# jabberjabberjabber/video-3d-pipeline

Hardware: AMD Instinct MI355X
Metric: 1080p_sbs_to_4k_depth_frames_per_s (higher is better)
Workload: dtype int16 (SGM) + f64 (guided filter sums; f32 depth in/out)

## Files before the change

video-3d-pipeline_amd/csrc/v3d_guided.hip:

```cpp
#include "v3d_common.h"
#include <type_traits>

__device__ __forceinline__ double gf_rcp(double x)
{
    double r = __builtin_amdgcn_rcp(x);
    r = fma(r, fma(-x, r, 1.0), r);
    r = fma(r, fma(-x, r, 1.0), r);
    return r;
}

template <typename TD> __device__ __forceinline__ float gf_ld(const TD* p, size_t i);
template <> __device__ __forceinline__ float gf_ld<float>(const float* p, size_t i) { return p[i]; }
template <> __device__ __forceinline__ float gf_ld<int16_t>(const int16_t* p, size_t i) { const int d = p[i]; return d > 0 ? (float)d * 0.0625f : 0.f; }

#define GF_TX 64
#define GF_RUN 8
#define GF_RMAX 16

template <typename TD>
__device__ __forceinline__ double gf_bilinear(const TD* __restrict__ src, int Ws, int Hs, double sx, double sy, int x, int y)
{
    const double fx = (x + 0.5) * sx - 0.5, fy = (y + 0.5) * sy - 0.5;
    const double x0f = floor(fx), y0f = floor(fy);
    const double wx = fx - x0f, wy = fy - y0f;
// ... 99 lines not shown
            }
            if (j + 1 < GF_RUNY) {
                const int kn = j + 2 * r + 1;
#pragma unroll
                for (int q = 0; q < NS; q++) s[q] += h[q * hplane + kn * hp] - h[q * hplane + j * hp];
            }
        }
    }
}

#ifndef GF_CH
#define GF_CH 3
#endif
typedef double v3d_f64x2 __attribute__((ext_vector_type(2)));
typedef float v3d_f32x2 __attribute__((ext_vector_type(2)));

template <int SWEEP, int RR, typename TD>
__global__ __launch_bounds__(256) void k_gfm(const TD* __restrict__ depth_lo, int Wlo, int Hlo,
                                             const uint8_t* __restrict__ guide, int W, int H, double eps, int band_h,
                                             double* __restrict__ A, double* __restrict__ B, float* __restrict__ out,
                                             size_t depth_stride, size_t guide_stride)
{
    static_assert(RR % 2 == 0, "pairs must not straddle the strip's halo boundary");
    constexpr int R = 2 * RR + 1, NOUT = 256 - 2 * RR;
    __shared__ __attribute__((aligned(16))) double sVd[2][2][2][256];
    __shared__ __attribute__((aligned(16))) int2 sVi[2][2][256];
    {
        const size_t f = blockIdx.z, n4 = (size_t)W * H;
        depth_lo += f * depth_stride; guide += f * guide_stride; A += f * 2 * n4; B += f * 2 * n4; out += f * n4;
    }
// ... 154 lines not shown
                                v3d_f32x2 vq = { qa, qb };
                                __builtin_nontemporal_store(vq, reinterpret_cast<v3d_f32x2*>(out + o));
                            } else {
                                out[o] = qa;
                                if (px1) out[o + 1] = qb;
                            }
                        }
                    }
                    buf ^= 1;
                }
            }
        }
    }
}

__device__ __forceinline__ double gf_partner(double v)
{
    const int lo = __builtin_amdgcn_update_dpp(0, __double2loint(v), V3D_DPP_QUAD(1, 0, 3, 2), 0xF, 0xF, true);
    const int hi = __builtin_amdgcn_update_dpp(0, __double2hiint(v), V3D_DPP_QUAD(1, 0, 3, 2), 0xF, 0xF, true);
    return __hiloint2double(hi, lo);
}
__device__ __forceinline__ int gf_partner(int v) { return __builtin_amdgcn_update_dpp(0, v, V3D_DPP_QUAD(1, 0, 3, 2), 0xF, 0xF, true); }

template <int RR, int COLS, typename TD, bool I1>
__global__ __launch_bounds__(2 * COLS, 4) void k_gff(const TD* __restrict__ depth_lo, int Wlo, int Hlo,
                                                const uint8_t* __restrict__ guide, int W, int H, double eps, int band_h,
                                                float* __restrict__ out, size_t depth_stride, size_t guide_stride)
{
    static_assert(RR % 2 == 0, "pairs must not straddle the strip's halo boundaries");
    static_assert(!I1 || std::is_same<TD, int16_t>::value, "the integer stage 1 takes the int16 disparity");
    constexpr int R = 2 * RR + 1, NOUT = COLS - 4 * RR, HP = COLS / 2;
    static_assert(COLS == 256 || COLS == 512, "strip width");
    constexpr int S1D = 2 * 2 * 2 * COLS * 8, S1I = 2 * 2 * COLS * 8;
    __shared__ __attribute__((aligned(16))) unsigned char sS1[I1 ? 2 * 2 * COLS * 16 : S1D + S1I];
    double (*sV1)[2][2][COLS] = reinterpret_cast<double (*)[2][2][COLS]>(sS1);
    int2 (*sVi)[2][COLS] = reinterpret_cast<int2 (*)[2][COLS]>(sS1 + (I1 ? 0 : S1D));
    int4 (*sVq)[2][COLS] = reinterpret_cast<int4 (*)[2][COLS]>(sS1);
    (void)sV1; (void)sVi; (void)sVq;
    __shared__ __attribute__((aligned(16))) double sAB[2][2][2][COLS];
    __shared__ __attribute__((aligned(16))) double sV2[2][2][2][COLS];
    __shared__ __attribute__((aligned(16))) double sP2[2][2][2][COLS / 2];
    __shared__ __attribute__((aligned(16))) int4 sPq[I1 ? 2 : 1][2][I1 ? COLS / 2 : 1];
    (void)sPq;
    {
        const size_t f = blockIdx.z, n4 = (size_t)W * H;
        depth_lo += f * depth_stride; guide += f * guide_stride; out += f * n4;
    }
    const int role = __builtin_amdgcn_readfirstlane((int)(threadIdx.x / COLS));
    const int t = threadIdx.x % COLS;
    const int gx0 = blockIdx.x * NOUT - 2 * RR;
    const int gx = gx0 + t;
    const int ya = blockIdx.y * band_h, yb = min(ya + band_h, H);
    const int nrows = (yb - ya) + 4 * RR;
    const int NS = (nrows + 1) >> 1;
    const int NP = NS + 3;
    const int hq = t % HP, hgx = gx0 + 2 * hq;

    for (int i = threadIdx.x; i < 2 * 2 * 2 * COLS; i += 2 * COLS) (&sAB[0][0][0][0])[i] = 0.0;
    __syncthreads();

    if (role == 0) {
      if constexpr (I1) {
        const bool col_ok = gx >= 0 && gx < W;
        const bool pair_in = 2 * hq >= RR && 2 * hq < COLS - RR;
        const bool px0 = pair_in && hgx >= 0 && hgx < W, px1 = pair_in && hgx + 1 >= 0 && hgx + 1 < W;
        const int kx = gx >> 1;
        const int bxa = min(max((gx & 1) ? kx : kx - 1, 0), Wlo - 1), bxb = min(max((gx & 1) ? kx + 1 : kx, 0), Wlo - 1);
        const int wxa = (gx & 1) ? 3 : 1, wxb = 4 - wxa;
        uint32_t ring[R];
        int vg = 0, vgg = 0, vP = 0, vgP = 0;
#pragma unroll
        for (int j = 0; j < R; j++) ring[j] = 0u;
        struct RowIn { int g, a0, a1, b0, b1; bool in; };
        const int gxc = min(max(gx, 0), W - 1);
        auto fetch_row = [&](int tt) -> RowIn {
            RowIn q;
            const int e = ya - 2 * RR + tt;
            q.in = col_ok && e >= 0 && e < H && tt < nrows;
            const int ec = min(max(e, 0), H - 1), ky = ec >> 1;
            q.g = guide[(size_t)ec * W + gxc];
            const TD* ra = depth_lo + (size_t)min(max((ec & 1) ? ky : ky - 1, 0), Hlo - 1) * Wlo;
            const TD* rb = depth_lo + (size_t)min(max((ec & 1) ? ky + 1 : ky, 0), Hlo - 1) * Wlo;
            q.a0 = max((int)ra[bxa], 0); q.a1 = max((int)ra[bxb], 0); q.b0 = max((int)rb[bxa], 0); q.b1 = max((int)rb[bxb], 0);
            return q;
        };
        RowIn nx[2] = { fetch_row(0), fetch_row(1) };
        for (int p0 = 0; p0 < NP; p0 += R) {
#pragma unroll
            for (int sp = 0; sp < R; sp++) {
                const int p = p0 + sp;
                if (p < NP) {
                    int tl = t;
                    asm volatile("" : "+v"(tl));
                    const int hrow = tl / HP, hq = tl % HP, hgx = gx0 + 2 * hq;
                    const int j = p - 1;
                    if (j >= RR && j < NS && pair_in) {
                        const int hb = j & 1;
                        const int y = ya - 3 * RR + 2 * j + hrow;
                        double ab[2][2] = { { 0.0, 0.0 }, { 0.0, 0.0 } };
                        if (y >= 0 && y < H && px0) {
                            const int4* gp = &sPq[hb][hrow][hq - RR / 2];
                            const int4 f = sVq[hb][hrow][2 * hq - RR], l = sVq[hb][hrow][2 * hq + RR + 1];
                            int4 c = make_int4(0, 0, 0, 0);
#pragma unroll
                            for (int ch = 0; ch <= RR; ch += 3) {
                                int4 u[3];
#pragma unroll
                                for (int i = 0; i < 3; i++) if (ch + i <= RR) u[i] = gp[ch + i];
#pragma unroll
                                for (int i = 0; i < 3; i++) if (ch + i <= RR) { c.x += u[i].x; c.y += u[i].y; c.z += u[i].z; c.w += u[i].w; }
                                asm volatile("" : "+v"(c.x), "+v"(c.y), "+v"(c.z), "+v"(c.w) :: "memory");
                            }
                            const int cy = min(y + RR, H - 1) - max(y - RR, 0) + 1;
                            const int cx0 = min(hgx + RR, W - 1) - max(hgx - RR, 0) + 1, cx1 = min(hgx + 1 + RR, W - 1) - max(hgx + 1 - RR, 0) + 1;
                            const double inva = gf_rcp((double)(cx0 * cy)), invb = cx1 == cx0 ? inva : gf_rcp((double)(cx1 * cy));
#pragma unroll
                            for (int n = 0; n < 2; n++) {
                                const int4 e = n ? f : l;
                                const double inv = n ? invb : inva;
                                const double s0 = (double)(c.z - e.z) * (1.0 / 256.0), s1 = (double)(c.w - e.w) * (1.0 / 256.0);
                                const double mI = (double)(c.x - e.x) * (inv * (1.0 / 255.0)), mp = s0 * inv;
                                const double mII = (double)(c.y - e.y) * (inv * (1.0 / 65025.0)), mIp = s1 * (inv * (1.0 / 255.0));
                                const double var = fma(-mI, mI, mII), cov = fma(-mI, mp, mIp);
                                const double a = cov * gf_rcp(var + eps);
                                ab[n][0] = a; ab[n][1] = fma(-a, mI, mp);
                            }
                            if (!px1) { ab[1][0] = 0.0; ab[1][1] = 0.0; }
                        }
                        const v3d_f64x2 va2 = { ab[0][0], ab[1][0] }, vb2 = { ab[0][1], ab[1][1] };
                        *reinterpret_cast<v3d_f64x2*>(&sAB[hb][hrow][0][2 * hq]) = va2;
                        *reinterpret_cast<v3d_f64x2*>(&sAB[hb][hrow][1][2 * hq]) = vb2;
                    }
                    if (p < NS) {
                        const int tA = 2 * p;
                        const RowIn cur[2] = { nx[0], nx[1] };
                        nx[0] = fetch_row(tA + 2); nx[1] = fetch_row(tA + 3);
                        const bool emit = p >= RR;
#pragma unroll
                        for (int rr = 0; rr < 2; rr++) {
                            const int slot = (2 * sp + rr) % R;
                            int gn = 0, Pn = 0;
                            if (cur[rr].in) {
                                gn = cur[rr].g;
                                const int e = ya - 2 * RR + tA + rr;
                                const int wya = (e & 1) ? 3 : 1;
                                Pn = wya * (wxa * cur[rr].a0 + wxb * cur[rr].a1) + (4 - wya) * (wxa * cur[rr].b0 + wxb * cur[rr].b1);
                            }
                            const int go = (int)(ring[slot] & 0xFFu), Po = (int)(ring[slot] >> 8);
                            ring[slot] = ((uint32_t)Pn << 8) | (uint32_t)gn;
                            vg += gn - go; vgg += gn * gn - go * go;
                            vP += Pn - Po; vgP += gn * Pn - go * Po;
                            if (emit) {
                                sVq[p & 1][rr][t] = make_int4(vg, vgg, vP, vgP);
                                const int4 ps = make_int4(vg + gf_partner(vg), vgg + gf_partner(vgg), vP + gf_partner(vP), vgP + gf_partner(vgP));
                                if (!(t & 1)) sPq[p & 1][rr][t >> 1] = ps;
                            }
                        }
                    }
                    __syncthreads();
                }
            }
        }
      } else {
        const bool col_ok = gx >= 0 && gx < W;
        const double sx = (double)Wlo / (double)W, sy = (double)Hlo / (double)H;
        const bool pair_in = 2 * hq >= RR && 2 * hq < COLS - RR;
        const bool px0 = pair_in && hgx >= 0 && hgx < W, px1 = pair_in && hgx + 1 >= 0 && hgx + 1 < W;
        int bxa, bxb; double bwx;
        {
            const double fx = (gx + 0.5) * sx - 0.5, x0f = floor(fx);
            bwx = fx - x0f;
            bxa = min(max((int)x0f, 0), Wlo - 1); bxb = min(max((int)x0f + 1, 0), Wlo - 1);
        }
        double r1[R], v0 = 0.0, v1 = 0.0;
        uint32_t rgw[(R + 3) / 4];
        int vg = 0, vgg = 0;
#pragma unroll
        for (int j = 0; j < R; j++) r1[j] = 0.0;
#pragma unroll
        for (int j = 0; j < (R + 3) / 4; j++) rgw[j] = 0u;
        struct RowIn { int g; float a0, a1, b0, b1; bool in; };
        const int gxc = min(max(gx, 0), W - 1);
        auto fetch_row = [&](int tt) -> RowIn {
            RowIn q;
            const int e = ya - 2 * RR + tt;
            q.in = col_ok && e >= 0 && e < H && tt < nrows;
            const size_t o = (size_t)min(max(e, 0), H - 1) * W + gxc;
            q.g = guide[o];
            const double fy = (e + 0.5) * sy - 0.5, y0f = floor(fy);
            const TD* ra = depth_lo + (size_t)min(max((int)y0f, 0), Hlo - 1) * Wlo;
            const TD* rb = depth_lo + (size_t)min(max((int)y0f + 1, 0), Hlo - 1) * Wlo;
            q.a0 = gf_ld(ra, bxa); q.a1 = gf_ld(ra, bxb); q.b0 = gf_ld(rb, bxa); q.b1 = gf_ld(rb, bxb);
            return q;
        };
        RowIn nx[2] = { fetch_row(0), fetch_row(1) };
        for (int p0 = 0; p0 < NP; p0 += R) {
#pragma unroll
            for (int sp = 0; sp < R; sp++) {
                const int p = p0 + sp;
                if (p < NP) {
                    int tl = t;
                    asm volatile("" : "+v"(tl));
                    const int hrow = tl / HP, hq = tl % HP, hgx = gx0 + 2 * hq;
                    const int j = p - 1;
                    if (j >= RR && j < NS && pair_in) {
                        const int hb = j & 1;
                        const int y = ya - 3 * RR + 2 * j + hrow;
                        double ab[2][2] = { { 0.0, 0.0 }, { 0.0, 0.0 } };
                        if (y >= 0 && y < H && px0) {
                            double fq[2], lq[2], cq[2];
#pragma unroll
                            for (int q = 0; q < 2; q++) {
                                const v3d_f64x2* d = reinterpret_cast<const v3d_f64x2*>(&sV1[hb][hrow][q][0]) + (hq - RR / 2);
                                double f = 0.0, l = 0.0, c = 0.0;
#pragma unroll
                                for (int ch = 0; ch <= RR; ch += GF_CH) {
                                    v3d_f64x2 w[GF_CH];
#pragma unroll
                                    for (int i = 0; i < GF_CH; i++) if (ch + i <= RR) w[i] = d[ch + i];
#pragma unroll
                                    for (int i = 0; i < GF_CH; i++) if (ch + i <= RR) {
                                        if (ch + i == 0) { f = w[i].x; c = w[i].y; }
                                        else if (ch + i == RR) { c += w[i].x; l = w[i].y; }
                                        else { c += w[i].x; c += w[i].y; }
                                    }
                                    asm volatile("" : "+v"(c) :: "memory");
                                }
                                fq[q] = f; lq[q] = l; cq[q] = c;
                            }
                            int g0 = 0, gg0 = 0, gl = 0, ggl = 0, cg = 0, cgg = 0;
                            {
                                const int4* gi = reinterpret_cast<const int4*>(&sVi[hb][hrow][0]) + (hq - RR / 2);
#pragma unroll
                                for (int ch = 0; ch <= RR; ch += 3) {
                                    int4 u[3];
#pragma unroll
                                    for (int i = 0; i < 3; i++) if (ch + i <= RR) u[i] = gi[ch + i];
#pragma unroll
                                    for (int i = 0; i < 3; i++) if (ch + i <= RR) {
                                        if (ch + i == 0) { g0 = u[i].x; gg0 = u[i].y; cg = u[i].z; cgg = u[i].w; }
                                        else if (ch + i == RR) { cg += u[i].x; cgg += u[i].y; gl = u[i].z; ggl = u[i].w; }
                                        else { cg += u[i].x + u[i].z; cgg += u[i].y + u[i].w; }
                                    }
                                    asm volatile("" : "+v"(cg), "+v"(cgg) :: "memory");
                                }
                            }
                            const double s0a = cq[0] + fq[0], s0b = cq[0] + lq[0], s1a = cq[1] + fq[1], s1b = cq[1] + lq[1];
                            const int cy = min(y + RR, H - 1) - max(y - RR, 0) + 1;
                            const int cx0 = min(hgx + RR, W - 1) - max(hgx - RR, 0) + 1, cx1 = min(hgx + 1 + RR, W - 1) - max(hgx + 1 - RR, 0) + 1;
                            const double inva = gf_rcp((double)(cx0 * cy)), invb = cx1 == cx0 ? inva : gf_rcp((double)(cx1 * cy));
                            const int sga = cg + g0, sgb = cg + gl, sgga = cgg + gg0, sggb = cgg + ggl;
#pragma unroll
                            for (int n = 0; n < 2; n++) {
                                const double inv = n ? invb : inva;
                                const double mI = (double)(n ? sgb : sga) * (inv * (1.0 / 255.0)), mp = (n ? s0b : s0a) * inv;
                                const double mII = (double)(n ? sggb : sgga) * (inv * (1.0 / 65025.0)), mIp = (n ? s1b : s1a) * (inv * (1.0 / 255.0));
                                const double var = fma(-mI, mI, mII), cov = fma(-mI, mp, mIp);
                                const double a = cov * gf_rcp(var + eps);
                                ab[n][0] = a; ab[n][1] = fma(-a, mI, mp);
                            }
                            if (!px1) { ab[1][0] = 0.0; ab[1][1] = 0.0; }
                        }
                        const v3d_f64x2 va2 = { ab[0][0], ab[1][0] }, vb2 = { ab[0][1], ab[1][1] };
                        *reinterpret_cast<v3d_f64x2*>(&sAB[hb][hrow][0][2 * hq]) = va2;
                        *reinterpret_cast<v3d_f64x2*>(&sAB[hb][hrow][1][2 * hq]) = vb2;
                    }
                    if (p < NS) {
                        const int tA = 2 * p;
                        const RowIn cur[2] = { nx[0], nx[1] };
                        nx[0] = fetch_row(tA + 2); nx[1] = fetch_row(tA + 3);
                        const bool emit = p >= RR;
#pragma unroll
                        for (int rr = 0; rr < 2; rr++) {
                            const int slot = (2 * sp + rr) % R;
                            int gn = 0; double pn = 0.0;
                            if (cur[rr].in) {
                                gn = cur[rr].g;
                                const int e = ya - 2 * RR + tA + rr;
                                const double fy = (e + 0.5) * sy - 0.5, wy = fy - floor(fy);
                                const double a0 = (double)cur[rr].a0, b0 = (double)cur[rr].b0;
                                const double top = fma(bwx, (double)cur[rr].a1 - a0, a0);
                                const double bot = fma(bwx, (double)cur[rr].b1 - b0, b0);
                                pn = fma(wy, bot - top, top);
                            }
                            const int go = (int)((rgw[slot >> 2] >> (8 * (slot & 3))) & 0xFFu); const double po = r1[slot];
                            rgw[slot >> 2] = (rgw[slot >> 2] & ~(0xFFu << (8 * (slot & 3)))) | ((uint32_t)gn << (8 * (slot & 3)));
                            r1[slot] = pn;
                            vg += gn - go; vgg += gn * gn - go * go;
                            v0 += pn - po; v1 = fma((double)gn, pn, fma(-(double)go, po, v1));
                            if (emit) {
                                sV1[p & 1][rr][0][t] = v0; sV1[p & 1][rr][1][t] = v1;
                                sVi[p & 1][rr][t] = make_int2(vg, vgg);
                            }
                        }
                    }
                    __syncthreads();
                }
            }
        }
      }
    } else {
        const bool pair_out = 2 * hq >= 2 * RR && 2 * hq < COLS - 2 * RR;
        const bool px0 = pair_out && hgx < W, px1 = pair_out && hgx + 1 < W;
        const bool vec_ok = px1 && (W & 1) == 0;
        double r0[R], r1[R], va = 0.0, vb = 0.0;
#pragma unroll
        for (int j = 0; j < R; j++) { r0[j] = 0.0; r1[j] = 0.0; }
        for (int p0 = 0; p0 < NP; p0 += R) {
#pragma unroll
            for (int sp = 0; sp < R; sp++) {
                const int p = p0 + sp;
                if (p < NP) {
                    int tl = t;
                    asm volatile("" : "+v"(tl));
                    const int hrow = tl / HP, hq = tl % HP, hgx = gx0 + 2 * hq;
                    {
                        const int j = p - 3;
                        const int y = ya - 4 * RR + 2 * j + hrow;
                        if (j >= 2 * RR && j < NS && px0 && y < yb) {
                            const int hb = j & 1;
                            double wa[2], wb[2];
#pragma unroll
                            for (int q = 0; q < 2; q++) {
                                const double* d = &sP2[hb][hrow][q][hq - RR / 2];
                                const double f = sV2[hb][hrow][q][2 * hq - RR], l = sV2[hb][hrow][q][2 * hq + RR + 1];
                                double c = 0.0;
#pragma unroll
                                for (int ch = 0; ch <= RR; ch += 3) {
                                    double w[3];
#pragma unroll
                                    for (int i = 0; i < 3; i++) if (ch + i <= RR) w[i] = d[ch + i];
#pragma unroll
                                    for (int i = 0; i < 3; i++) if (ch + i <= RR) c += w[i];
                                    asm volatile("" : "+v"(c) :: "memory");
                                }
                                wa[q] = c - l; wb[q] = c - f;
                                asm volatile("" : "+v"(wa[q]), "+v"(wb[q]) :: "memory");
                            }
                            const double s0a = wa[0], s0b = wb[0], s1a = wa[1], s1b = wb[1];
                            const int cy = min(y + RR, H - 1) - max(y - RR, 0) + 1;
                            const int cx0 = min(hgx + RR, W - 1) - max(hgx - RR, 0) + 1, cx1 = min(hgx + 1 + RR, W - 1) - max(hgx + 1 - RR, 0) + 1;
                            const double inva = gf_rcp((double)(cx0 * cy)), invb = cx1 == cx0 ? inva : gf_rcp((double)(cx1 * cy));
                            const size_t o = (size_t)y * W + hgx;
                            const double Ia = (double)guide[o] * (1.0 / 255.0);
                            const double Ib = px1 ? (double)guide[o + 1] * (1.0 / 255.0) : 0.0;
                            const float qa = (float)((s0a * inva) * Ia + (s1a * inva)), qb = (float)((s0b * invb) * Ib + (s1b * invb));
                            if (vec_ok) {
                                v3d_f32x2 vq = { qa, qb };
                                __builtin_nontemporal_store(vq, reinterpret_cast<v3d_f32x2*>(out + o));
                            } else {
                                out[o] = qa;
                                if (px1) out[o + 1] = qb;
                            }
                        }
                    }
                    {
                        const int j = p - 2;
                        if (j >= RR && j < NS) {
                            const bool emit = j >= 2 * RR;
#pragma unroll
                            for (int rr = 0; rr < 2; rr++) {
                                const int slot = (2 * sp + rr) % R;
                                const double n0 = sAB[j & 1][rr][0][tl], n1 = sAB[j & 1][rr][1][tl];
                                const double o0 = r0[slot], o1 = r1[slot];
                                r0[slot] = n0; r1[slot] = n1;
                                va += n0 - o0; vb += n1 - o1;
                                if (emit) {
                                    sV2[j & 1][rr][0][tl] = va; sV2[j & 1][rr][1][tl] = vb;
                                    const double pa = va + gf_partner(va), pb = vb + gf_partner(vb);
                                    if (!(tl & 1)) { sP2[j & 1][rr][0][tl >> 1] = pa; sP2[j & 1][rr][1][tl >> 1] = pb; }
                                }
                            }
                        }
                    }
                    __syncthreads();
                }
            }
        }
    }
}

template <int RR, typename TD>
static void launch_gff(const TD* depth_lo, int Wlo, int Hlo, const uint8_t* guide, int W, int H, double eps,
                       float* out, int n, size_t depth_stride, size_t guide_stride, hipStream_t st)
{
    const int cols = g_v3d_opt.gf_cols == 512 ? 512 : 256;
    int band = g_v3d_opt.gf_band;
    if (band <= 0) {
        int dev = 0, ncu = 256;
        (void)hipGetDevice(&dev);
        (void)hipDeviceGetAttribute(&ncu, hipDeviceAttributeMultiprocessorCount, dev);
        const long slots = (long)ncu * (cols == 512 ? 1 : 2), strips = v3d_cdiv(W, cols - 4 * RR);
        long best = -1;
        for (int nb = 1; nb <= 64 && nb <= H; nb++) {
            const int b = (v3d_cdiv(H, nb) + 1) & ~1;
            const long wgs = strips * v3d_cdiv(H, b) * n, rounds = (wgs + slots - 1) / slots, cost = rounds * (b + 4 * RR);
            if (best < 0 || cost < best) { best = cost; band = b; }
        }
    }
    if (g_v3d_opt.gf_cols == 512) {
        const dim3 grid(v3d_cdiv(W, 512 - 4 * RR), v3d_cdiv(H, band), n);
        hipLaunchKernelGGL((k_gff<RR, 512, TD, false>), grid, dim3(1024), 0, st, depth_lo, Wlo, Hlo, guide, W, H, eps, band, out, depth_stride, guide_stride);
        return;
    }
    const dim3 grid(v3d_cdiv(W, 256 - 4 * RR), v3d_cdiv(H, band), n);
    if constexpr (std::is_same<TD, int16_t>::value) {
        if (g_v3d_opt.gf_int1 && W == 2 * Wlo && H == 2 * Hlo) {
            hipLaunchKernelGGL((k_gff<RR, 256, TD, true>), grid, dim3(512), 0, st, depth_lo, Wlo, Hlo, guide, W, H, eps, band, out, depth_stride, guide_stride);
            return;
        }
    }
    hipLaunchKernelGGL((k_gff<RR, 256, TD, false>), grid, dim3(512), 0, st, depth_lo, Wlo, Hlo, guide, W, H, eps, band, out, depth_stride, guide_stride);
}

template <int RR, typename TD>
static void launch_gfm(const TD* depth_lo, int Wlo, int Hlo, const uint8_t* guide, int W, int H, double eps,
                       double* A, double* B, float* out, int n, size_t depth_stride, size_t guide_stride, hipStream_t st)
{
    const int band1 = g_v3d_opt.gf_band1, band2 = g_v3d_opt.gf_band2;
    const dim3 grid1(v3d_cdiv(W, 256 - 2 * RR), v3d_cdiv(H, band1), n), grid2(v3d_cdiv(W, 256 - 2 * RR), v3d_cdiv(H, band2), n);
    hipLaunchKernelGGL((k_gfm<1, RR, TD>), grid1, dim3(256), 0, st, depth_lo, Wlo, Hlo, guide, W, H, eps, band1, A, B, out, depth_stride, guide_stride);
    hipLaunchKernelGGL((k_gfm<2, RR, TD>), grid2, dim3(256), 0, st, depth_lo, Wlo, Hlo, guide, W, H, eps, band2, A, B, out, depth_stride, guide_stride);
// ... 79 lines not shown
```

Measured before the change: 2485.

## Process four rows and four-pixel runs per step in fused guided filter

Restructures the fused guided-filter kernel so each step handles four rows and each thread computes a run of four horizontal box sums, using swizzled LDS layouts to avoid bank conflicts. The paired DPP partner-sum scheme and the separate sV2/sP2 buffers are replaced by a triple-buffered sAB array reused in place. The aim is fewer barriers per row and fewer LDS reads per output. It costs more registers and LDS, lowers the occupancy hint for the f64 route, and limits 512-column strips to the integer path.

```diff
diff --git a/video-3d-pipeline_amd/csrc/v3d_guided.hip b/video-3d-pipeline_amd/csrc/v3d_guided.hip
--- a/video-3d-pipeline_amd/csrc/v3d_guided.hip
+++ b/video-3d-pipeline_amd/csrc/v3d_guided.hip
@@ -137,6 +137,7 @@
 #endif
 typedef double v3d_f64x2 __attribute__((ext_vector_type(2)));
 typedef float v3d_f32x2 __attribute__((ext_vector_type(2)));
+typedef float v3d_f32x4 __attribute__((ext_vector_type(4)));
 
 template <int SWEEP, int RR, typename TD>
 __global__ __launch_bounds__(256) void k_gfm(const TD* __restrict__ depth_lo, int Wlo, int Hlo,
@@ -321,34 +322,128 @@
     }
 }
 
-__device__ __forceinline__ double gf_partner(double v)
-{
-    const int lo = __builtin_amdgcn_update_dpp(0, __double2loint(v), V3D_DPP_QUAD(1, 0, 3, 2), 0xF, 0xF, true);
-    const int hi = __builtin_amdgcn_update_dpp(0, __double2hiint(v), V3D_DPP_QUAD(1, 0, 3, 2), 0xF, 0xF, true);
-    return __hiloint2double(hi, lo);
-}
-__device__ __forceinline__ int gf_partner(int v) { return __builtin_amdgcn_update_dpp(0, v, V3D_DPP_QUAD(1, 0, 3, 2), 0xF, 0xF, true); }
+__device__ __forceinline__ int gf_swz2(int m) { return m ^ ((m >> 3) & 1) ^ ((m >> 4) & 1); }
+__device__ __forceinline__ int gf_swz4(int m) { return m ^ ((m >> 4) & 3); }
+__device__ __forceinline__ int gf_c8(int c) { return 2 * gf_swz2(c >> 1) + (c & 1); }
+
+template <int RR>
+__device__ __forceinline__ void gf_run4(const double* row, int c0, double s[4])
+{
+    const v3d_f64x2* d = reinterpret_cast<const v3d_f64x2*>(row);
+    const int m0 = (c0 - RR) >> 1;
+    double c = 0.0, l0 = 0.0, l1 = 0.0, l2 = 0.0, r1 = 0.0, r2 = 0.0, r3 = 0.0;
+#pragma unroll
+    for (int k0 = 0; k0 < RR + 2; k0 += GF_CH) {
+        v3d_f64x2 w[GF_CH];
+#pragma unroll
+        for (int i = 0; i < GF_CH; i++) if (k0 + i < RR + 2) w[i] = d[gf_swz2(m0 + k0 + i)];
+#pragma unroll
+        for (int i = 0; i < GF_CH; i++) {
+            const int k = k0 + i;
+            if (k == 0) { l0 = w[i].x; l1 = w[i].y; c = w[i].x; c += w[i].y; }
+            else if (k == 1) { l2 = w[i].x; c += w[i].x; c += w[i].y; }
+            else if (k < RR) { c += w[i].x; c += w[i].y; }
+            else if (k == RR) { c += w[i].x; r1 = w[i].y; }
+            else if (k == RR + 1) { r2 = w[i].x; r3 = w[i].y; }
+        }
+        asm volatile("" : "+v"(c) :: "memory");
+    }
+    s[0] = c; s[1] = (s[0] + r1) - l0; s[2] = (s[1] + r2) - l1; s[3] = (s[2] + r3) - l2;
+}
+
+template <int RR>
+__device__ __forceinline__ void gf_run4(const int2* row, int c0, int2 s[4])
+{
+    const int4* d = reinterpret_cast<const int4*>(row);
+    const int m0 = (c0 - RR) >> 1;
+    int2 c = make_int2(0, 0), l0 = c, l1 = c, l2 = c, r1 = c, r2 = c, r3 = c;
+#pragma unroll
+    for (int k0 = 0; k0 < RR + 2; k0 += 3) {
+        int4 w[3];
+#pragma unroll
+        for (int i = 0; i < 3; i++) if (k0 + i < RR + 2) w[i] = d[gf_swz2(m0 + k0 + i)];
+#pragma unroll
+        for (int i = 0; i < 3; i++) {
+            const int k = k0 + i;
+            const int2 a = make_int2(w[i].x, w[i].y), b = make_int2(w[i].z, w[i].w);
+            if (k == 0) { l0 = a; l1 = b; c = make_int2(a.x + b.x, a.y + b.y); }
+            else if (k == 1) { l2 = a; c.x += a.x + b.x; c.y += a.y + b.y; }
+            else if (k < RR) { c.x += a.x + b.x; c.y += a.y + b.y; }
+            else if (k == RR) { c.x += a.x; c.y += a.y; r1 = b; }
+            else if (k == RR + 1) { r2 = a; r3 = b; }
+        }
+        asm volatile("" : "+v"(c.x), "+v"(c.y) :: "memory");
+    }
+    s[0] = c;
+    s[1] = make_int2(s[0].x + r1.x - l0.x, s[0].y + r1.y - l0.y);
+    s[2] = make_int2(s[1].x + r2.x - l1.x, s[1].y + r2.y - l1.y);
+    s[3] = make_int2(s[2].x + r3.x - l2.x, s[2].y + r3.y - l2.y);
+}
+
+template <int RR>
+__device__ __forceinline__ void gf_run4(const int4* row, int c0, int4 s[4])
+{
+    int4 c = make_int4(0, 0, 0, 0), l0 = c, l1 = c, l2 = c, r1 = c, r2 = c, r3 = c;
+#pragma unroll
+    for (int k0 = 0; k0 < 2 * RR + 4; k0 += 3) {
+        int4 u[3];
+#pragma unroll
+        for (int i = 0; i < 3; i++) if (k0 + i < 2 * RR + 4) u[i] = row[gf_swz4(c0 - RR + k0 + i)];
+#pragma unroll
+        for (int i = 0; i < 3; i++) {
+            const int k = k0 + i;
+            if (k < 2 * RR + 1) { c.x += u[i].x; c.y += u[i].y; c.z += u[i].z; c.w += u[i].w; }
+            if (k == 0) l0 = u[i];
+            else if (k == 1) l1 = u[i];
+            else if (k == 2) l2 = u[i];
+            else if (k == 2 * RR + 1) r1 = u[i];
+            else if (k == 2 * RR + 2) r2 = u[i];
+            else if (k == 2 * RR + 3) r3 = u[i];
+        }
+        asm volatile("" : "+v"(c.x), "+v"(c.y), "+v"(c.z), "+v"(c.w) :: "memory");
+    }
+    s[0] = c;
+    s[1] = make_int4(s[0].x + r1.x - l0.x, s[0].y + r1.y - l0.y, s[0].z + r1.z - l0.z, s[0].w + r1.w - l0.w);
+    s[2] = make_int4(s[1].x + r2.x - l1.x, s[1].y + r2.y - l1.y, s[1].z + r2.z - l1.z, s[1].w + r2.w - l1.w);
+    s[3] = make_int4(s[2].x + r3.x - l2.x, s[2].y + r3.y - l2.y, s[2].z + r3.z - l2.z, s[2].w + r3.w - l2.w);
+}
+
+template <int RR>
+__device__ __forceinline__ void gf_solve4(const int sg[4], const int sgg[4], const double sp[4], const double sgp[4], int hgx, int y,
+                                          int W, int H, double eps, double a[4], double b[4])
+{
+    const int cy = min(y + RR, H - 1) - max(y - RR, 0) + 1;
+    int cx[4];
+#pragma unroll
+    for (int n = 0; n < 4; n++) cx[n] = min(hgx + n + RR, W - 1) - max(hgx + n - RR, 0) + 1;
+    const double inv0 = gf_rcp((double)(cx[0] * cy));
+#pragma unroll
+    for (int n = 0; n < 4; n++) {
+        const double inv = (n == 0 || cx[n] == cx[0]) ? inv0 : gf_rcp((double)(cx[n] * cy));
+        const double mI = (double)sg[n] * (inv * (1.0 / 255.0)), mp = sp[n] * inv;
+        const double mII = (double)sgg[n] * (inv * (1.0 / 65025.0)), mIp = sgp[n] * (inv * (1.0 / 255.0));
+        const double var = fma(-mI, mI, mII), cov = fma(-mI, mp, mIp);
+        const double aa = cov * gf_rcp(var + eps);
+        a[n] = aa; b[n] = fma(-aa, mI, mp);
+    }
+}
 
 template <int RR, int COLS, typename TD, bool I1>
-__global__ __launch_bounds__(2 * COLS, 4) void k_gff(const TD* __restrict__ depth_lo, int Wlo, int Hlo,
+__global__ __launch_bounds__(2 * COLS, I1 ? 4 : 2) void k_gff(const TD* __restrict__ depth_lo, int Wlo, int Hlo,
                                                 const uint8_t* __restrict__ guide, int W, int H, double eps, int band_h,
                                                 float* __restrict__ out, size_t depth_stride, size_t guide_stride)
 {
-    static_assert(RR % 2 == 0, "pairs must not straddle the strip's halo boundaries");
+    static_assert(RR % 4 == 0, "runs of four must not straddle the strip's halo boundaries");
     static_assert(!I1 || std::is_same<TD, int16_t>::value, "the integer stage 1 takes the int16 disparity");
-    constexpr int R = 2 * RR + 1, NOUT = COLS - 4 * RR, HP = COLS / 2;
-    static_assert(COLS == 256 || COLS == 512, "strip width");
-    constexpr int S1D = 2 * 2 * 2 * COLS * 8, S1I = 2 * 2 * COLS * 8;
-    __shared__ __attribute__((aligned(16))) unsigned char sS1[I1 ? 2 * 2 * COLS * 16 : S1D + S1I];
-    double (*sV1)[2][2][COLS] = reinterpret_cast<double (*)[2][2][COLS]>(sS1);
-    int2 (*sVi)[2][COLS] = reinterpret_cast<int2 (*)[2][COLS]>(sS1 + (I1 ? 0 : S1D));
-    int4 (*sVq)[2][COLS] = reinterpret_cast<int4 (*)[2][COLS]>(sS1);
+    static_assert(COLS == 256 || (COLS == 512 && I1), "strip width (512 columns: I1 only, the f64 route's rows exceed the LDS)");
+    constexpr int R = 2 * RR + 1, NOUT = COLS - 4 * RR, HR = COLS / 4;
+    constexpr int S1D = 2 * 4 * 2 * COLS * 8, S1 = I1 ? 2 * 4 * COLS * 16 : S1D + 2 * 4 * COLS * 8;
+    __shared__ __attribute__((aligned(16))) unsigned char sS1[S1];
+    double (*sV1)[4][2][COLS] = reinterpret_cast<double (*)[4][2][COLS]>(sS1);
+    int2 (*sVi)[4][COLS] = reinterpret_cast<int2 (*)[4][COLS]>(sS1 + (I1 ? 0 : S1D));
+    int4 (*sVq)[4][COLS] = reinterpret_cast<int4 (*)[4][COLS]>(sS1);
     (void)sV1; (void)sVi; (void)sVq;
-    __shared__ __attribute__((aligned(16))) double sAB[2][2][2][COLS];
-    __shared__ __attribute__((aligned(16))) double sV2[2][2][2][COLS];
-    __shared__ __attribute__((aligned(16))) double sP2[2][2][2][COLS / 2];
-    __shared__ __attribute__((aligned(16))) int4 sPq[I1 ? 2 : 1][2][I1 ? COLS / 2 : 1];
-    (void)sPq;
+    __shared__ __attribute__((aligned(16))) double sAB[3][4][2][COLS];
     {
         const size_t f = blockIdx.z, n4 = (size_t)W * H;
         depth_lo += f * depth_stride; guide += f * guide_stride; out += f * n4;
@@ -359,108 +454,140 @@
     const int gx = gx0 + t;
     const int ya = blockIdx.y * band_h, yb = min(ya + band_h, H);
     const int nrows = (yb - ya) + 4 * RR;
-    const int NS = (nrows + 1) >> 1;
+    const int NS = (nrows + 3) >> 2;
     const int NP = NS + 3;
-    const int hq = t % HP, hgx = gx0 + 2 * hq;
-
-    for (int i = threadIdx.x; i < 2 * 2 * 2 * COLS; i += 2 * COLS) (&sAB[0][0][0][0])[i] = 0.0;
-    __syncthreads();
 
     if (role == 0) {
-      if constexpr (I1) {
         const bool col_ok = gx >= 0 && gx < W;
-        const bool pair_in = 2 * hq >= RR && 2 * hq < COLS - RR;
-        const bool px0 = pair_in && hgx >= 0 && hgx < W, px1 = pair_in && hgx + 1 >= 0 && hgx + 1 < W;
-        const int kx = gx >> 1;
-        const int bxa = min(max((gx & 1) ? kx : kx - 1, 0), Wlo - 1), bxb = min(max((gx & 1) ? kx + 1 : kx, 0), Wlo - 1);
-        const int wxa = (gx & 1) ? 3 : 1, wxb = 4 - wxa;
+        const int gxc = min(max(gx, 0), W - 1);
         uint32_t ring[R];
+        double r1[I1 ? 1 : R];
+        uint32_t rgw[I1 ? 1 : (R + 3) / 4];
         int vg = 0, vgg = 0, vP = 0, vgP = 0;
+        double v0 = 0.0, v1 = 0.0;
 #pragma unroll
         for (int j = 0; j < R; j++) ring[j] = 0u;
-        struct RowIn { int g, a0, a1, b0, b1; bool in; };
-        const int gxc = min(max(gx, 0), W - 1);
+#pragma unroll
+        for (int j = 0; j < (I1 ? 1 : R); j++) r1[j] = 0.0;
+#pragma unroll
+        for (int j = 0; j < (I1 ? 1 : (R + 3) / 4); j++) rgw[j] = 0u;
+        (void)ring; (void)r1; (void)rgw;
+        int bxa, bxb, wxa = 0, wxb = 0; double bwx = 0.0;
+        const double sx = (double)Wlo / (double)W, sy = (double)Hlo / (double)H;
+        if constexpr (I1) {
+            const int kx = gx >> 1;
+            bxa = min(max((gx & 1) ? kx : kx - 1, 0), Wlo - 1); bxb = min(max((gx & 1) ? kx + 1 : kx, 0), Wlo - 1);
+            wxa = (gx & 1) ? 3 : 1; wxb = 4 - wxa;
+        } else {
+            const double fx = (gx + 0.5) * sx - 0.5, x0f = floor(fx);
+            bwx = fx - x0f;
+            bxa = min(max((int)x0f, 0), Wlo - 1); bxb = min(max((int)x0f + 1, 0), Wlo - 1);
+        }
+        (void)wxa; (void)wxb; (void)bwx;
+        struct RowIn { int g; typename std::conditional<I1, int, float>::type a0, a1, b0, b1; bool in; };
         auto fetch_row = [&](int tt) -> RowIn {
             RowIn q;
             const int e = ya - 2 * RR + tt;
             q.in = col_ok && e >= 0 && e < H && tt < nrows;
-            const int ec = min(max(e, 0), H - 1), ky = ec >> 1;
+            const int ec = min(max(e, 0), H - 1);
             q.g = guide[(size_t)ec * W + gxc];
-            const TD* ra = depth_lo + (size_t)min(max((ec & 1) ? ky : ky - 1, 0), Hlo - 1) * Wlo;
-            const TD* rb = depth_lo + (size_t)min(max((ec & 1) ? ky + 1 : ky, 0), Hlo - 1) * Wlo;
-            q.a0 = max((int)ra[bxa], 0); q.a1 = max((int)ra[bxb], 0); q.b0 = max((int)rb[bxa], 0); q.b1 = max((int)rb[bxb], 0);
+            if constexpr (I1) {
+                const int ky = ec >> 1;
+                const TD* ra = depth_lo + (size_t)min(max((ec & 1) ? ky : ky - 1, 0), Hlo - 1) * Wlo;
+                const TD* rb = depth_lo + (size_t)min(max((ec & 1) ? ky + 1 : ky, 0), Hlo - 1) * Wlo;
+                q.a0 = max((int)ra[bxa], 0); q.a1 = max((int)ra[bxb], 0); q.b0 = max((int)rb[bxa], 0); q.b1 = max((int)rb[bxb], 0);
+            } else {
+                const double fy = (e + 0.5) * sy - 0.5, y0f = floor(fy);
+                const TD* ra = depth_lo + (size_t)min(max((int)y0f, 0), Hlo - 1) * Wlo;
+                const TD* rb = depth_lo + (size_t)min(max((int)y0f + 1, 0), Hlo - 1) * Wlo;
+                q.a0 = gf_ld(ra, bxa); q.a1 = gf_ld(ra, bxb); q.b0 = gf_ld(rb, bxa); q.b1 = gf_ld(rb, bxb);
+            }
             return q;
         };
-        RowIn nx[2] = { fetch_row(0), fetch_row(1) };
+        RowIn nx[4] = { fetch_row(0), fetch_row(1), fetch_row(2), fetch_row(3) };
         for (int p0 = 0; p0 < NP; p0 += R) {
-#pragma unroll
+#pragma clang loop unroll(full)
             for (int sp = 0; sp < R; sp++) {
                 const int p = p0 + sp;
                 if (p < NP) {
                     int tl = t;
                     asm volatile("" : "+v"(tl));
-                    const int hrow = tl / HP, hq = tl % HP, hgx = gx0 + 2 * hq;
+                    const int hrow = tl / HR, c0 = 4 * (tl % HR), hgx = gx0 + c0;
                     const int j = p - 1;
-                    if (j >= RR && j < NS && pair_in) {
-                        const int hb = j & 1;
-                        const int y = ya - 3 * RR + 2 * j + hrow;
-                        double ab[2][2] = { { 0.0, 0.0 }, { 0.0, 0.0 } };
-                        if (y >= 0 && y < H && px0) {
-                            const int4* gp = &sPq[hb][hrow][hq - RR / 2];
-                            const int4 f = sVq[hb][hrow][2 * hq - RR], l = sVq[hb][hrow][2 * hq + RR + 1];
-                            int4 c = make_int4(0, 0, 0, 0);
-#pragma unroll
-                            for (int ch = 0; ch <= RR; ch += 3) {
-                                int4 u[3];
-#pragma unroll
-                                for (int i = 0; i < 3; i++) if (ch + i <= RR) u[i] = gp[ch + i];
-#pragma unroll
-                                for (int i = 0; i < 3; i++) if (ch + i <= RR) { c.x += u[i].x; c.y += u[i].y; c.z += u[i].z; c.w += u[i].w; }
-                                asm volatile("" : "+v"(c.x), "+v"(c.y), "+v"(c.z), "+v"(c.w) :: "memory");
-                            }
-                            const int cy = min(y + RR, H - 1) - max(y - RR, 0) + 1;
-                            const int cx0 = min(hgx + RR, W - 1) - max(hgx - RR, 0) + 1, cx1 = min(hgx + 1 + RR, W - 1) - max(hgx + 1 - RR, 0) + 1;
-                            const double inva = gf_rcp((double)(cx0 * cy)), invb = cx1 == cx0 ? inva : gf_rcp((double)(cx1 * cy));
-#pragma unroll
-                            for (int n = 0; n < 2; n++) {
-                                const int4 e = n ? f : l;
-                                const double inv = n ? invb : inva;
-                                const double s0 = (double)(c.z - e.z) * (1.0 / 256.0), s1 = (double)(c.w - e.w) * (1.0 / 256.0);
-                                const double mI = (double)(c.x - e.x) * (inv * (1.0 / 255.0)), mp = s0 * inv;
-                                const double mII = (double)(c.y - e.y) * (inv * (1.0 / 65025.0)), mIp = s1 * (inv * (1.0 / 255.0));
-                                const double var = fma(-mI, mI, mII), cov = fma(-mI, mp, mIp);
-                                const double a = cov * gf_rcp(var + eps);
-                                ab[n][0] = a; ab[n][1] = fma(-a, mI, mp);
-                            }
-                            if (!px1) { ab[1][0] = 0.0; ab[1][1] = 0.0; }
+                    if (j >= RR / 2 && j < NS) {
+                        const int y = ya - 3 * RR + 4 * j + hrow;
+                        double a[4] = { 0.0, 0.0, 0.0, 0.0 }, b[4] = { 0.0, 0.0, 0.0, 0.0 };
+                        if (c0 >= RR && c0 < COLS - RR && y >= 0 && y < H && hgx >= 0 && hgx < W) {
+                            int sg[4], sgg[4]; double sp_[4], sgp[4];
+                            if constexpr (I1) {
+                                int4 s[4];
+                                gf_run4<RR>(&sVq[j & 1][hrow][0], c0, s);
+#pragma unroll
+                                for (int n = 0; n < 4; n++) {
+                                    sg[n] = s[n].x; sgg[n] = s[n].y;
+                                    sp_[n] = (double)s[n].z * (1.0 / 256.0); sgp[n] = (double)s[n].w * (1.0 / 256.0);
+                                }
+                            } else {
+                                int2 si[4];
+                                gf_run4<RR>(&sVi[j & 1][hrow][0], c0, si);
+                                gf_run4<RR>(&sV1[j & 1][hrow][0][0], c0, sp_);
+                                gf_run4<RR>(&sV1[j & 1][hrow][1][0], c0, sgp);
+#pragma unroll
+                                for (int n = 0; n < 4; n++) { sg[n] = si[n].x; sgg[n] = si[n].y; }
+                            }
+                            gf_solve4<RR>(sg, sgg, sp_, sgp, hgx, y, W, H, eps, a, b);
+#pragma unroll
+                            for (int n = 0; n < 4; n++) if (hgx + n >= W) { a[n] = 0.0; b[n] = 0.0; }
                         }
-                        const v3d_f64x2 va2 = { ab[0][0], ab[1][0] }, vb2 = { ab[0][1], ab[1][1] };
-                        *reinterpret_cast<v3d_f64x2*>(&sAB[hb][hrow][0][2 * hq]) = va2;
-                        *reinterpret_cast<v3d_f64x2*>(&sAB[hb][hrow][1][2 * hq]) = vb2;
+                        double* ab = &sAB[j % 3][hrow][0][0];
+                        const int e0 = 2 * gf_swz2(c0 >> 1), e1 = 2 * gf_swz2((c0 >> 1) + 1);
+                        *reinterpret_cast<v3d_f64x2*>(ab + e0) = v3d_f64x2{ a[0], a[1] };
+                        *reinterpret_cast<v3d_f64x2*>(ab + e1) = v3d_f64x2{ a[2], a[3] };
+                        *reinterpret_cast<v3d_f64x2*>(ab + COLS + e0) = v3d_f64x2{ b[0], b[1] };
+                        *reinterpret_cast<v3d_f64x2*>(ab + COLS + e1) = v3d_f64x2{ b[2], b[3] };
                     }
                     if (p < NS) {
-                        const int tA = 2 * p;
-                        const RowIn cur[2] = { nx[0], nx[1] };
-                        nx[0] = fetch_row(tA + 2); nx[1] = fetch_row(tA + 3);
-                        const bool emit = p >= RR;
-#pragma unroll
-                        for (int rr = 0; rr < 2; rr++) {
-                            const int slot = (2 * sp + rr) % R;
-                            int gn = 0, Pn = 0;
-                            if (cur[rr].in) {
-                                gn = cur[rr].g;
-                                const int e = ya - 2 * RR + tA + rr;
-                                const int wya = (e & 1) ? 3 : 1;
-                                Pn = wya * (wxa * cur[rr].a0 + wxb * cur[rr].a1) + (4 - wya) * (wxa * cur[rr].b0 + wxb * cur[rr].b1);
-                            }
-                            const int go = (int)(ring[slot] & 0xFFu), Po = (int)(ring[slot] >> 8);
-                            ring[slot] = ((uint32_t)Pn << 8) | (uint32_t)gn;
-                            vg += gn - go; vgg += gn * gn - go * go;
-                            vP += Pn - Po; vgP += gn * Pn - go * Po;
-                            if (emit) {
-                                sVq[p & 1][rr][t] = make_int4(vg, vgg, vP, vgP);
-                                const int4 ps = make_int4(vg + gf_partner(vg), vgg + gf_partner(vgg), vP + gf_partner(vP), vgP + gf_partner(vgP));
-                                if (!(t & 1)) sPq[p & 1][rr][t >> 1] = ps;
+                        const int tA = 4 * p;
+                        const RowIn cur[4] = { nx[0], nx[1], nx[2], nx[3] };
+#pragma unroll
+                        for (int k = 0; k < 4; k++) nx[k] = fetch_row(tA + 4 + k);
+                        const bool emit = p >= RR / 2;
+#pragma unroll
+                        for (int rr = 0; rr < 4; rr++) {
+                            const int slot = (4 * sp + rr) % R;
+                            const int e = ya - 2 * RR + tA + rr;
+                            if constexpr (I1) {
+                                int gn = 0, Pn = 0;
+                                if (cur[rr].in) {
+                                    gn = cur[rr].g;
+                                    const int wya = (e & 1) ? 3 : 1;
+                                    Pn = wya * (wxa * cur[rr].a0 + wxb * cur[rr].a1) + (4 - wya) * (wxa * cur[rr].b0 + wxb * cur[rr].b1);
+                                }
+                                const int go = (int)(ring[slot] & 0xFFu), Po = (int)(ring[slot] >> 8);
+                                ring[slot] = ((uint32_t)Pn << 8) | (uint32_t)gn;
+                                vg += gn - go; vgg += gn * gn - go * go;
+                                vP += Pn - Po; vgP += gn * Pn - go * Po;
+                                if (emit) sVq[p & 1][rr][gf_swz4(t)] = make_int4(vg, vgg, vP, vgP);
+                            } else {
+                                int gn = 0; double pn = 0.0;
+                                if (cur[rr].in) {
+                                    gn = cur[rr].g;
+                                    const double fy = (e + 0.5) * sy - 0.5, wy = fy - floor(fy);
+                                    const double a0 = (double)cur[rr].a0, b0 = (double)cur[rr].b0;
+                                    const double top = fma(bwx, (double)cur[rr].a1 - a0, a0);
+                                    const double bot = fma(bwx, (double)cur[rr].b1 - b0, b0);
+                                    pn = fma(wy, bot - top, top);
+                                }
+                                const int go = (int)((rgw[slot >> 2] >> (8 * (slot & 3))) & 0xFFu); const double po = r1[slot];
+                                rgw[slot >> 2] = (rgw[slot >> 2] & ~(0xFFu << (8 * (slot & 3)))) | ((uint32_t)gn << (8 * (slot & 3)));
+                                r1[slot] = pn;
+                                vg += gn - go; vgg += gn * gn - go * go;
+                                v0 += pn - po; v1 = fma((double)gn, pn, fma(-(double)go, po, v1));
+                                if (emit) {
+                                    const int ct = gf_c8(t);
+                                    sV1[p & 1][rr][0][ct] = v0; sV1[p & 1][rr][1][ct] = v1;
+                                    sVi[p & 1][rr][ct] = make_int2(vg, vgg);
+                                }
                             }
                         }
                     }
@@ -468,136 +595,72 @@
                 }
             }
         }
-      } else {
-        const bool col_ok = gx >= 0 && gx < W;
-        const double sx = (double)Wlo / (double)W, sy = (double)Hlo / (double)H;
-        const bool pair_in = 2 * hq >= RR && 2 * hq < COLS - RR;
-        const bool px0 = pair_in && hgx >= 0 && hgx < W, px1 = pair_in && hgx + 1 >= 0 && hgx + 1 < W;
-        int bxa, bxb; double bwx;
-        {
-            const double fx = (gx + 0.5) * sx - 0.5, x0f = floor(fx);
-            bwx = fx - x0f;
-            bxa = min(max((int)x0f, 0), Wlo - 1); bxb = min(max((int)x0f + 1, 0), Wlo - 1);
-        }
-        double r1[R], v0 = 0.0, v1 = 0.0;
-        uint32_t rgw[(R + 3) / 4];
-        int vg = 0, vgg = 0;
-#pragma unroll
-        for (int j = 0; j < R; j++) r1[j] = 0.0;
-#pragma unroll
-        for (int j = 0; j < (R + 3) / 4; j++) rgw[j] = 0u;
-        struct RowIn { int g; float a0, a1, b0, b1; bool in; };
-        const int gxc = min(max(gx, 0), W - 1);
-        auto fetch_row = [&](int tt) -> RowIn {
-            RowIn q;
-            const int e = ya - 2 * RR + tt;
-            q.in = col_ok && e >= 0 && e < H && tt < nrows;
-            const size_t o = (size_t)min(max(e, 0), H - 1) * W + gxc;
-            q.g = guide[o];
-            const double fy = (e + 0.5) * sy - 0.5, y0f = floor(fy);
-            const TD* ra = depth_lo + (size_t)min(max((int)y0f, 0), Hlo - 1) * Wlo;
-            const TD* rb = depth_lo + (size_t)min(max((int)y0f + 1, 0), Hlo - 1) * Wlo;
-            q.a0 = gf_ld(ra, bxa); q.a1 = gf_ld(ra, bxb); q.b0 = gf_ld(rb, bxa); q.b1 = gf_ld(rb, bxb);
-            return q;
-        };
-        RowIn nx[2] = { fetch_row(0), fetch_row(1) };
+    } else {
+        double r0[R], r1[R], va = 0.0, vb = 0.0;
+#pragma unroll
+        for (int j = 0; j < R; j++) { r0[j] = 0.0; r1[j] = 0.0; }
         for (int p0 = 0; p0 < NP; p0 += R) {
-#pragma unroll
+#pragma clang loop unroll(full)
             for (int sp = 0; sp < R; sp++) {
                 const int p = p0 + sp;
                 if (p < NP) {
                     int tl = t;
                     asm volatile("" : "+v"(tl));
-                    const int hrow = tl / HP, hq = tl % HP, hgx = gx0 + 2 * hq;
-                    const int j = p - 1;
-                    if (j >= RR && j < NS && pair_in) {
-                        const int hb = j & 1;
-                        const int y = ya - 3 * RR + 2 * j + hrow;
-                        double ab[2][2] = { { 0.0, 0.0 }, { 0.0, 0.0 } };
-                        if (y >= 0 && y < H && px0) {
-                            double fq[2], lq[2], cq[2];
-#pragma unroll
-                            for (int q = 0; q < 2; q++) {
-                                const v3d_f64x2* d = reinterpret_cast<const v3d_f64x2*>(&sV1[hb][hrow][q][0]) + (hq - RR / 2);
-                                double f = 0.0, l = 0.0, c = 0.0;
-#pragma unroll
-                                for (int ch = 0; ch <= RR; ch += GF_CH) {
-                                    v3d_f64x2 w[GF_CH];
-#pragma unroll
-                                    for (int i = 0; i < GF_CH; i++) if (ch + i <= RR) w[i] = d[ch + i];
-#pragma unroll
-                                    for (int i = 0; i < GF_CH; i++) if (ch + i <= RR) {
-                                        if (ch + i == 0) { f = w[i].x; c = w[i].y; }
-                                        else if (ch + i == RR) { c += w[i].x; l = w[i].y; }
-                                        else { c += w[i].x; c += w[i].y; }
-                                    }
-                                    asm volatile("" : "+v"(c) :: "memory");
-                                }
-                                fq[q] = f; lq[q] = l; cq[q] = c;
-                            }
-                            int g0 = 0, gg0 = 0, gl = 0, ggl = 0, cg = 0, cgg = 0;
-                            {
-                                const int4* gi = reinterpret_cast<const int4*>(&sVi[hb][hrow][0]) + (hq - RR / 2);
-#pragma unroll
-                                for (int ch = 0; ch <= RR; ch += 3) {
-                                    int4 u[3];
-#pragma unroll
-                                    for (int i = 0; i < 3; i++) if (ch + i <= RR) u[i] = gi[ch + i];
-#pragma unroll
-                                    for (int i = 0; i < 3; i++) if (ch + i <= RR) {
-                                        if (ch + i == 0) { g0 = u[i].x; gg0 = u[i].y; cg = u[i].z; cgg = u[i].w; }
-                                        else if (ch + i == RR) { cg += u[i].x; cgg += u[i].y; gl = u[i].z; ggl = u[i].w; }
-                                        else { cg += u[i].x + u[i].z; cgg += u[i].y + u[i].w; }
-                                    }
-                                    asm volatile("" : "+v"(cg), "+v"(cgg) :: "memory");
-                                }
-                            }
-                            const double s0a = cq[0] + fq[0], s0b = cq[0] + lq[0], s1a = cq[1] + fq[1], s1b = cq[1] + lq[1];
+                    const int hrow = tl / HR, c0 = 4 * (tl % HR), hgx = gx0 + c0;
+                    {
+                        const int j = p - 3;
+                        const int y = ya - 4 * RR + 4 * j + hrow;
+                        if (j >= RR && j < NS && c0 >= 2 * RR && c0 < COLS - 2 * RR && hgx < W && y < yb) {
+                            double sa[4], sb[4];
+                            gf_run4<RR>(&sAB[j % 3][hrow][0][0], c0, sa);
+                            gf_run4<RR>(&sAB[j % 3][hrow][1][0], c0, sb);
                             const int cy = min(y + RR, H - 1) - max(y - RR, 0) + 1;
-                            const int cx0 = min(hgx + RR, W - 1) - max(hgx - RR, 0) + 1, cx1 = min(hgx + 1 + RR, W - 1) - max(hgx + 1 - RR, 0) + 1;
-                            const double inva = gf_rcp((double)(cx0 * cy)), invb = cx1 == cx0 ? inva : gf_rcp((double)(cx1 * cy));
-                            const int sga = cg + g0, sgb = cg + gl, sgga = cgg + gg0, sggb = cgg + ggl;
-#pragma unroll
-                            for (int n = 0; n < 2; n++) {
-                                const double inv = n ? invb : inva;
-                                const double mI = (double)(n ? sgb : sga) * (inv * (1.0 / 255.0)), mp = (n ? s0b : s0a) * inv;
-                                const double mII = (double)(n ? sggb : sgga) * (inv * (1.0 / 65025.0)), mIp = (n ? s1b : s1a) * (inv * (1.0 / 255.0));
-                                const double var = fma(-mI, mI, mII), cov = fma(-mI, mp, mIp);
-                                const double a = cov * gf_rcp(var + eps);
-                                ab[n][0] = a; ab[n][1] = fma(-a, mI, mp);
-                            }
-                            if (!px1) { ab[1][0] = 0.0; ab[1][1] = 0.0; }
+                            int cx[4];
+#pragma unroll
+                            for (int n = 0; n < 4; n++) cx[n] = min(hgx + n + RR, W - 1) - max(hgx + n - RR, 0) + 1;
+                            const double inv0 = gf_rcp((double)(cx[0] * cy));
+                            const size_t o = (size_t)y * W + hgx;
+                            const bool all_in = hgx + 3 < W;
+                            const bool vec_ok = all_in && (W & 3) == 0 && ((reinterpret_cast<uintptr_t>(out + o) | reinterpret_cast<uintptr_t>(guide + o)) & 3) == 0
+                                                && (reinterpret_cast<uintptr_t>(out + o) & 15) == 0;
+                            int g[4];
+                            if (vec_ok) {
+                                const uint32_t g4 = *reinterpret_cast<const uint32_t*>(guide + o);
+#pragma unroll
+                                for (int n = 0; n < 4; n++) g[n] = (g4 >> (8 * n)) & 0xFF;
+                            } else {
+#pragma unroll
+                                for (int n = 0; n < 4; n++) g[n] = hgx + n < W ? guide[o + n] : 0;
+                            }
+                            float q[4];
+#pragma unroll
+                            for (int n = 0; n < 4; n++) {
+                                const double inv = (n == 0 || cx[n] == cx[0]) ? inv0 : gf_rcp((double)(cx[n] * cy));
+                                const double I = (double)g[n] * (1.0 / 255.0);
+                                q[n] = (float)((sa[n] * inv) * I + (sb[n] * inv));
+                            }
+                            if (vec_ok) {
+                                const v3d_f32x4 vq = { q[0], q[1], q[2], q[3] };
+                                __builtin_nontemporal_store(vq, reinterpret_cast<v3d_f32x4*>(out + o));
+                            } else {
+#pragma unroll
+                                for (int n = 0; n < 4; n++) if (hgx + n < W) out[o + n] = q[n];
+                            }
                         }
-                        const v3d_f64x2 va2 = { ab[0][0], ab[1][0] }, vb2 = { ab[0][1], ab[1][1] };
-                        *reinterpret_cast<v3d_f64x2*>(&sAB[hb][hrow][0][2 * hq]) = va2;
-                        *reinterpret_cast<v3d_f64x2*>(&sAB[hb][hrow][1][2 * hq]) = vb2;
                     }
-                    if (p < NS) {
-                        const int tA = 2 * p;
-                        const RowIn cur[2] = { nx[0], nx[1] };
-                        nx[0] = fetch_row(tA + 2); nx[1] = fetch_row(tA + 3);
-                        const bool emit = p >= RR;
-#pragma unroll
-                        for (int rr = 0; rr < 2; rr++) {
-                            const int slot = (2 * sp + rr) % R;
-                            int gn = 0; double pn = 0.0;
-                            if (cur[rr].in) {
-                                gn = cur[rr].g;
-                                const int e = ya - 2 * RR + tA + rr;
-                                const double fy = (e + 0.5) * sy - 0.5, wy = fy - floor(fy);
-                                const double a0 = (double)cur[rr].a0, b0 = (double)cur[rr].b0;
-                                const double top = fma(bwx, (double)cur[rr].a1 - a0, a0);
-                                const double bot = fma(bwx, (double)cur[rr].b1 - b0, b0);
-                                pn = fma(wy, bot - top, top);
-                            }
-                            const int go = (int)((rgw[slot >> 2] >> (8 * (slot & 3))) & 0xFFu); const double po = r1[slot];
-                            rgw[slot >> 2] = (rgw[slot >> 2] & ~(0xFFu << (8 * (slot & 3)))) | ((uint32_t)gn << (8 * (slot & 3)));
-                            r1[slot] = pn;
-                            vg += gn - go; vgg += gn * gn - go * go;
-                            v0 += pn - po; v1 = fma((double)gn, pn, fma(-(double)go, po, v1));
-                            if (emit) {
-                                sV1[p & 1][rr][0][t] = v0; sV1[p & 1][rr][1][t] = v1;
-                                sVi[p & 1][rr][t] = make_int2(vg, vgg);
+                    {
+                        const int j = p - 2;
+                        if (j >= RR / 2 && j < NS) {
+                            const bool emit = j >= RR;
+                            double* col = &sAB[j % 3][0][0][gf_c8(tl)];
+#pragma unroll
+                            for (int rr = 0; rr < 4; rr++) {
+                                const int slot = (4 * sp + rr) % R;
+                                const double n0 = col[rr * 2 * COLS], n1 = col[rr * 2 * COLS + COLS];
+                                const double o0 = r0[slot], o1 = r1[slot];
+                                r0[slot] = n0; r1[slot] = n1;
+                                va += n0 - o0; vb += n1 - o1;
+                                if (emit) { col[rr * 2 * COLS] = va; col[rr * 2 * COLS + COLS] = vb; }
                             }
                         }
                     }
@@ -605,85 +668,6 @@
                 }
             }
         }
-      }
-    } else {
-        const bool pair_out = 2 * hq >= 2 * RR && 2 * hq < COLS - 2 * RR;
-        const bool px0 = pair_out && hgx < W, px1 = pair_out && hgx + 1 < W;
-        const bool vec_ok = px1 && (W & 1) == 0;
-        double r0[R], r1[R], va = 0.0, vb = 0.0;
-#pragma unroll
-        for (int j = 0; j < R; j++) { r0[j] = 0.0; r1[j] = 0.0; }
-        for (int p0 = 0; p0 < NP; p0 += R) {
-#pragma unroll
-            for (int sp = 0; sp < R; sp++) {
-                const int p = p0 + sp;
-                if (p < NP) {
-                    int tl = t;
-                    asm volatile("" : "+v"(tl));
-                    const int hrow = tl / HP, hq = tl % HP, hgx = gx0 + 2 * hq;
-                    {
-                        const int j = p - 3;
-                        const int y = ya - 4 * RR + 2 * j + hrow;
-                        if (j >= 2 * RR && j < NS && px0 && y < yb) {
-                            const int hb = j & 1;
-                            double wa[2], wb[2];
-#pragma unroll
-                            for (int q = 0; q < 2; q++) {
-                                const double* d = &sP2[hb][hrow][q][hq - RR / 2];
-                                const double f = sV2[hb][hrow][q][2 * hq - RR], l = sV2[hb][hrow][q][2 * hq + RR + 1];
-                                double c = 0.0;
-#pragma unroll
-                                for (int ch = 0; ch <= RR; ch += 3) {
-                                    double w[3];
-#pragma unroll
-                                    for (int i = 0; i < 3; i++) if (ch + i <= RR) w[i] = d[ch + i];
-#pragma unroll
-                                    for (int i = 0; i < 3; i++) if (ch + i <= RR) c += w[i];
-                                    asm volatile("" : "+v"(c) :: "memory");
-                                }
-                                wa[q] = c - l; wb[q] = c - f;
-                                asm volatile("" : "+v"(wa[q]), "+v"(wb[q]) :: "memory");
-                            }
-                            const double s0a = wa[0], s0b = wb[0], s1a = wa[1], s1b = wb[1];
-                            const int cy = min(y + RR, H - 1) - max(y - RR, 0) + 1;
-                            const int cx0 = min(hgx + RR, W - 1) - max(hgx - RR, 0) + 1, cx1 = min(hgx + 1 + RR, W - 1) - max(hgx + 1 - RR, 0) + 1;
-                            const double inva = gf_rcp((double)(cx0 * cy)), invb = cx1 == cx0 ? inva : gf_rcp((double)(cx1 * cy));
-                            const size_t o = (size_t)y * W + hgx;
-                            const double Ia = (double)guide[o] * (1.0 / 255.0);
-                            const double Ib = px1 ? (double)guide[o + 1] * (1.0 / 255.0) : 0.0;
-                            const float qa = (float)((s0a * inva) * Ia + (s1a * inva)), qb = (float)((s0b * invb) * Ib + (s1b * invb));
-                            if (vec_ok) {
-                                v3d_f32x2 vq = { qa, qb };
-                                __builtin_nontemporal_store(vq, reinterpret_cast<v3d_f32x2*>(out + o));
-                            } else {
-                                out[o] = qa;
-                                if (px1) out[o + 1] = qb;
-                            }
-                        }
-                    }
-                    {
-                        const int j = p - 2;
-                        if (j >= RR && j < NS) {
-                            const bool emit = j >= 2 * RR;
-#pragma unroll
-                            for (int rr = 0; rr < 2; rr++) {
-                                const int slot = (2 * sp + rr) % R;
-                                const double n0 = sAB[j & 1][rr][0][tl], n1 = sAB[j & 1][rr][1][tl];
-                                const double o0 = r0[slot], o1 = r1[slot];
-                                r0[slot] = n0; r1[slot] = n1;
-                                va += n0 - o0; vb += n1 - o1;
-                                if (emit) {
-                                    sV2[j & 1][rr][0][tl] = va; sV2[j & 1][rr][1][tl] = vb;
-                                    const double pa = va + gf_partner(va), pb = vb + gf_partner(vb);
-                                    if (!(tl & 1)) { sP2[j & 1][rr][0][tl >> 1] = pa; sP2[j & 1][rr][1][tl >> 1] = pb; }
-                                }
-                            }
-                        }
-                    }
-                    __syncthreads();
-                }
-            }
-        }
     }
 }
 
@@ -691,13 +675,15 @@
 static void launch_gff(const TD* depth_lo, int Wlo, int Hlo, const uint8_t* guide, int W, int H, double eps,
                        float* out, int n, size_t depth_stride, size_t guide_stride, hipStream_t st)
 {
-    const int cols = g_v3d_opt.gf_cols == 512 ? 512 : 256;
+    bool i1 = false;
+    if constexpr (std::is_same<TD, int16_t>::value) i1 = g_v3d_opt.gf_int1 && W == 2 * Wlo && H == 2 * Hlo;
+    const int cols = g_v3d_opt.gf_cols == 512 && i1 ? 512 : 256;
     int band = g_v3d_opt.gf_band;
     if (band <= 0) {
         int dev = 0, ncu = 256;
         (void)hipGetDevice(&dev);
         (void)hipDeviceGetAttribute(&ncu, hipDeviceAttributeMultiprocessorCount, dev);
-        const long slots = (long)ncu * (cols == 512 ? 1 : 2), strips = v3d_cdiv(W, cols - 4 * RR);
+        const long slots = (long)ncu * (cols == 256 && i1 ? 2 : 1), strips = v3d_cdiv(W, cols - 4 * RR);
         long best = -1;
         for (int nb = 1; nb <= 64 && nb <= H; nb++) {
             const int b = (v3d_cdiv(H, nb) + 1) & ~1;
@@ -705,14 +691,13 @@
             if (best < 0 || cost < best) { best = cost; band = b; }
         }
     }
-    if (g_v3d_opt.gf_cols == 512) {
-        const dim3 grid(v3d_cdiv(W, 512 - 4 * RR), v3d_cdiv(H, band), n);
-        hipLaunchKernelGGL((k_gff<RR, 512, TD, false>), grid, dim3(1024), 0, st, depth_lo, Wlo, Hlo, guide, W, H, eps, band, out, depth_stride, guide_stride);
-        return;
-    }
-    const dim3 grid(v3d_cdiv(W, 256 - 4 * RR), v3d_cdiv(H, band), n);
+    const dim3 grid(v3d_cdiv(W, cols - 4 * RR), v3d_cdiv(H, band), n);
     if constexpr (std::is_same<TD, int16_t>::value) {
-        if (g_v3d_opt.gf_int1 && W == 2 * Wlo && H == 2 * Hlo) {
+        if (i1 && cols == 512) {
+            hipLaunchKernelGGL((k_gff<RR, 512, TD, true>), grid, dim3(1024), 0, st, depth_lo, Wlo, Hlo, guide, W, H, eps, band, out, depth_stride, guide_stride);
+            return;
+        }
+        if (i1) {
             hipLaunchKernelGGL((k_gff<RR, 256, TD, true>), grid, dim3(512), 0, st, depth_lo, Wlo, Hlo, guide, W, H, eps, band, out, depth_stride, guide_stride);
             return;
         }
```

Result: faster. 2592, median of 6 (+4.3%).
